# endernewton/tf-faster-rcnn

Hardware: NVIDIA H100
Metric: images/sec (higher is better)
Workload: dtype f16x3 (fp32-grade: fp16 hi/lo split of both operands, 3 wgmma f16 MMAs per product, fp32 accumulate)

## Files before the change

include/frcnn_b200.h:

```cpp
#ifndef FRCNN_B200_H_
#define FRCNN_B200_H_

#include <stddef.h>
#include <stdint.h>

#ifdef __cplusplus
extern "C" {
#endif

typedef enum {
  FRCNN_OK = 0,
  FRCNN_ERR_CUDA = -1,
  FRCNN_ERR_ARG = -2,
  FRCNN_ERR_NO_DEVICE = -3,
  FRCNN_ERR_DRIVER_ENTRY = -4,
  FRCNN_ERR_CAPACITY = -5
} frcnn_status;

#define FRCNN_NMS_PLUS_ONE 1u
#define FRCNN_NMS_INCLUSIVE 2u
#define FRCNN_NMS_SKIP_DEGENERATE 4u
#define FRCNN_NMS_MODE_CPU_NMS (FRCNN_NMS_PLUS_ONE | FRCNN_NMS_INCLUSIVE)
#define FRCNN_NMS_MODE_GPU_NMS (FRCNN_NMS_PLUS_ONE)
#define FRCNN_NMS_MODE_TF (FRCNN_NMS_SKIP_DEGENERATE)
// ... 16 lines not shown
int frcnn_nms_host(int* keep_out, int* num_out, const float* boxes_host, int boxes_num, int boxes_dim,
                   float nms_overlap_thresh, int device_id, unsigned flags);

int frcnn_nms_sorted_dev(const float* boxes_dev, int n, float thresh, unsigned flags, int max_out,
                         int* keep_dev, int* num_dev, void* stream);

typedef struct frcnn_conv_plan frcnn_conv_plan;
#define FRCNN_CONV_F16X3 0
#define FRCNN_CONV_TF32X3 1
#define FRCNN_CONV_F16X1 2

typedef struct {
  const float* in_dev;
  const void* w_hi_dev;
  const void* w_lo_dev;
  const float* scale_dev;
  const float* shift_dev;
  const float* residual_dev;
  float* out_dev;
  int n, h, w, cin;
  int cout, kh, kw, stride;
  int pad_t, pad_l;
  int ho, wo;
  int act;
  int block_n;
  int kb_per_chunk;
  int split_k;
  int impl;
  float out_mult;
  const float* in2_dev;
  int cin2;
  float* mean_dev;
  int mean_hw;
} frcnn_conv_desc;

int frcnn_conv_plan_create(frcnn_conv_plan** out, const frcnn_conv_desc* d);
int frcnn_conv_plan_run(const frcnn_conv_plan* p, void* stream);
int frcnn_conv_plan_geometry(const frcnn_conv_desc* d, int sm_count, int* out16);
int frcnn_conv_plan_info(const frcnn_conv_plan* p, int* block_n, int* tile_n, int* tile_h, int* tile_w,
                         int* grid_m, int* grid_n, int* splits, int* smem_bytes);
int frcnn_conv_plan_set_trace(frcnn_conv_plan* p, long long* trace_dev);
void frcnn_conv_plan_destroy(frcnn_conv_plan* p);
int frcnn_debug_watchdog(unsigned int* out16, int reset);

int frcnn_pack_conv_weights(const float* w_hwio_dev, void* w_hi_dev, void* w_lo_dev, int kh, int kw,
                            int cin, int cout, int wexp, void* stream);
int frcnn_pack_conv_weights_tf32(const float* w_hwio_dev, float* w_hi_dev, float* w_lo_dev, int kh, int kw,
                                 int cin, int cout, void* stream);

int frcnn_conv_first(const float* in_dev, const float* w_hwio_dev, const float* scale_dev,
                     const float* shift_dev, float* out_dev, int n, int h, int w, int cout, int k,
                     int stride, int pad_t, int pad_l, int ho, int wo, int act, void* stream);
int frcnn_depthwise3x3(const float* in_dev, const float* w_dev, const float* scale_dev,
                       const float* shift_dev, float* out_dev, int n, int h, int w, int c, int stride,
                       int pad_t, int pad_l, int ho, int wo, int act, void* stream);
int frcnn_max_pool(const float* in_dev, float* out_dev, int n, int h, int w, int c, int k, int stride,
                   int pad_t, int pad_l, int ho, int wo, int pad_is_neg_inf, void* stream);
int frcnn_spatial_mean(const float* in_dev, float* out_dev, int r, int hw, int c, void* stream);

int frcnn_preprocess(const unsigned char* img_dev, int h0, int w0, const double* means3, double fx, double fy,
                     float* blob_dev, int H, int W, void* stream);
int frcnn_preprocess_hflip(const unsigned char* img_dev, int h0, int w0, const double* means3, double fx, double fy,
                           float* blob_dev, int H, int W, void* stream);


int frcnn_rpn_decode(const float* rpn_out_dev, int ld, int delta_col, const float* base_anchors_dev, int num_anchors,
                     int batch, int fh, int fw, int feat_stride, float im_h, float im_w, float* scores_dev,
                     float* props_dev, void* stream);
size_t frcnn_sort_workspace_bytes(int n);
int frcnn_sort_desc(const float* keys_dev, int n, int batch, int* order_dev, float* sorted_keys_dev, void* workspace_dev,
                    size_t workspace_bytes, void* stream);
// ... 68 lines not shown
```

tf_faster_rcnn_b200/_native.py:

```python
import ctypes as C
import os

_HERE = os.path.dirname(os.path.abspath(__file__))
LIB_PATH = os.path.join(_HERE, "libfrcnn_b200_wd.so" if os.environ.get("FRCNN_LIB_VARIANT") == "wd" else "libfrcnn_b200.so")

NMS_PLUS_ONE, NMS_INCLUSIVE, NMS_SKIP_DEGENERATE = 1, 2, 4
NMS_MODE_CPU_NMS = NMS_PLUS_ONE | NMS_INCLUSIVE
NMS_MODE_GPU_NMS = NMS_PLUS_ONE
NMS_MODE_TF = NMS_SKIP_DEGENERATE
ACT_NONE, ACT_RELU, ACT_RELU6 = 0, 1, 2
CONV_F16X3, CONV_TF32X3, CONV_F16X1 = 0, 1, 2
SOFT_NMS_METHODS = {"linear": 0, "gaussian": 1, "hard": 2}
AUG_MAX_VIEWS = 16
BOX_VOTE_METHODS = {"ID": 0, "AVG": 1, "IOU_AVG": 2, "GENERALIZED_AVG": 3, "QUASI_SUM": 4, "TEMP_AVG": 5}
ROI_ALIGN_MAX_SAMPLING = 16
ROI_MAX_POOLED = 16

vp, ci, cf, cu, sz = C.c_void_p, C.c_int, C.c_float, C.c_uint, C.c_size_t
ip, fp = C.POINTER(C.c_int), C.POINTER(C.c_float)


class ConvDesc(C.Structure):
    _fields_ = [("in_dev", vp), ("w_hi_dev", vp), ("w_lo_dev", vp), ("scale_dev", vp), ("shift_dev", vp),
                ("residual_dev", vp), ("out_dev", vp),
                ("n", ci), ("h", ci), ("w", ci), ("cin", ci), ("cout", ci), ("kh", ci), ("kw", ci), ("stride", ci),
                ("pad_t", ci), ("pad_l", ci), ("ho", ci), ("wo", ci), ("act", ci), ("block_n", ci), ("kb_per_chunk", ci), ("split_k", ci),
                ("impl", ci), ("out_mult", cf), ("in2_dev", vp), ("cin2", ci), ("mean_dev", vp), ("mean_hw", ci)]


SIGNATURES = {
    "frcnn_version": (ci, []),
    "frcnn_last_error": (ci, [C.c_char_p, sz]),
    "frcnn_check_device": (ci, [ci]),
    "frcnn_zero_async": (ci, [vp, sz, vp]),
    "frcnn_graph_begin": (ci, [vp]),
    "frcnn_graph_end": (ci, [vp, C.POINTER(vp)]),
    "frcnn_graph_launch": (ci, [vp, vp]),
    "frcnn_graph_destroy": (None, [vp]),
    "frcnn_nms_host": (ci, [ip, ip, fp, ci, ci, cf, ci, cu]),
    "frcnn_nms_sorted_dev": (ci, [vp, ci, cf, cu, ci, vp, vp, vp]),
    "frcnn_conv_plan_create": (ci, [C.POINTER(vp), C.POINTER(ConvDesc)]),
    "frcnn_conv_plan_run": (ci, [vp, vp]),
    "frcnn_conv_plan_geometry": (ci, [C.POINTER(ConvDesc), ci, ip]),
    "frcnn_conv_plan_info": (ci, [vp, ip, ip, ip, ip, ip, ip, ip, ip]),
    "frcnn_conv_plan_set_trace": (ci, [vp, vp]),
    "frcnn_conv_plan_destroy": (None, [vp]),
    "frcnn_debug_watchdog": (ci, [C.POINTER(C.c_uint), ci]),
    "frcnn_pack_conv_weights": (ci, [vp, vp, vp, ci, ci, ci, ci, ci, vp]),
    "frcnn_pack_conv_weights_tf32": (ci, [vp, vp, vp, ci, ci, ci, ci, vp]),
    "frcnn_conv_first": (ci, [vp, vp, vp, vp, vp, ci, ci, ci, ci, ci, ci, ci, ci, ci, ci, ci, vp]),
    "frcnn_depthwise3x3": (ci, [vp, vp, vp, vp, vp, ci, ci, ci, ci, ci, ci, ci, ci, ci, ci, vp]),
    "frcnn_max_pool": (ci, [vp, vp, ci, ci, ci, ci, ci, ci, ci, ci, ci, ci, ci, vp]),
    "frcnn_spatial_mean": (ci, [vp, vp, ci, ci, ci, vp]),
    "frcnn_preprocess": (ci, [vp, ci, ci, C.POINTER(C.c_double), C.c_double, C.c_double, vp, ci, ci, vp]),
    "frcnn_rpn_decode": (ci, [vp, ci, ci, vp, ci, ci, ci, ci, ci, cf, cf, vp, vp, vp]),
    "frcnn_sort_workspace_bytes": (sz, [ci]),
    "frcnn_sort_desc": (ci, [vp, ci, ci, vp, vp, vp, sz, vp]),
    "frcnn_proposals": (ci, [vp, vp, vp, ci, ci, ci, ci, cf, cu, vp, vp, vp, vp, vp]),
    "frcnn_crop_pool": (ci, [vp, ci, ci, ci, ci, vp, ci, ci, ci, vp, vp]),
    "frcnn_roi_align": (ci, [vp, ci, ci, ci, ci, vp, ci, ci, cf, ci, ci, vp, vp]),
    "frcnn_roi_pool": (ci, [vp, ci, ci, ci, ci, vp, ci, ci, cf, vp, vp]),
    "frcnn_cls_finish": (ci, [vp, ci, ci, ci, fp, fp, vp, vp, vp, vp]),
    "frcnn_bbox_decode": (ci, [vp, vp, ci, ci, ci, vp, vp, vp]),
    "frcnn_detect_post_workspace_bytes": (sz, [ci, ci, ci]),
    "frcnn_detect_post": (ci, [vp, vp, vp, ci, ci, ci, cf, cf, cu, ci, ci, vp, vp, ci, vp, vp, vp, vp, sz, vp]),
    "frcnn_soft_nms_host": (ci, [fp, ip, ip, fp, ci, ci, ci, cf, cf, cf, ci]),
    "frcnn_detect_post_soft": (ci, [vp, vp, vp, ci, ci, ci, cf, ci, cf, cf, cf, ci, ci, vp, vp, ci, vp, vp, vp, vp, sz, vp]),
    "frcnn_detect_features": (ci, [vp, vp, vp, ci, ci, ci, ci, ci, vp, vp, vp]),
    "frcnn_detect_regions": (ci, [vp, vp, vp, vp, vp, ci, ci, ci, ci, cf, cu, cf, ci, ci, vp, vp, vp, vp, sz, vp, vp, vp, vp, vp, vp, vp,
                                  vp, vp]),
    "frcnn_boxes_to_rois": (ci, [vp, vp, vp, ci, ci, vp, vp, vp]),
    "frcnn_preprocess_hflip": (ci, [vp, ci, ci, C.POINTER(C.c_double), C.c_double, C.c_double, vp, ci, ci, vp]),
    "frcnn_aug_union": (ci, [C.POINTER(vp), C.POINTER(vp), C.POINTER(vp), ip, ip, ci, ci, ci, vp, vp, vp, vp, vp]),
    "frcnn_box_vote_host": (ci, [fp, fp, ci, ci, fp, ci, ci, cf, ci, cf, ci]),
    "frcnn_detect_post_vote": (ci, [vp, vp, vp, ci, ci, ci, cf, cf, cu, ci, ci, vp, vp, ci, vp, vp, vp, vp, sz, cf, ci, cf, vp, vp]),
    "frcnn_detect_post_soft_vote": (ci, [vp, vp, vp, ci, ci, ci, cf, ci, cf, cf, cf, ci, ci, vp, vp, ci, vp, vp, vp, vp, sz, cf, ci, cf, vp,
# ... 31 lines not shown
```

tf_faster_rcnn_b200/csrc/conv_gemm.cu:

```cuda
#include <cuda_fp16.h>
#include "common.cuh"
#include "../../include/frcnn_b200.h"
#include <stdlib.h>
#include <string.h>

namespace frcnn {

constexpr int BLOCK_M = 128;
constexpr int BLOCK_K = 32;
constexpr int A_TILE_BYTES = BLOCK_M * BLOCK_K * 4;
constexpr int NUM_CONSUMERS = 256;
constexpr int NUM_THREADS = NUM_CONSUMERS + 128;
constexpr int REGS_PRODUCER = 40, REGS_CONSUMER = 232;
constexpr int STAGES = 3;

struct ConvKernelParams {
  float* out;
  const float* residual;
  const float* scale;
  const float* shift;
  int cout, ho, wo, nimg;
  int tn, th, tw;
  int tiles_h, tiles_w;
  int kh, kw, cin, stride, pad_t, pad_l;
  int act;
  int a_box_bytes;
  int kb_per_split;
  int m_tiles, n_tiles, total_units, n_full, splits;
  int raster_n;
  float* ws;
  long long* trace;
  int num_kb_total;
  int cin2;
  float* mean_out;
  float* mean_ws;
  int mean_hw, mean_segs, mean_ld;
};

#ifdef FRCNN_WATCHDOG
#define FRCNN_TRACE(slot, kbv)                                                              \
  do {                                                                                      \
    if (p.trace && blockIdx.x == 0 && (kbv) < 64) p.trace[(kbv) * 8 + (slot)] = clock64(); \
  } while (0)
#else
#define FRCNN_TRACE(slot, kbv) do { } while (0)
#endif

template <int MODE> struct KTraits {
  static constexpr bool TF32 = MODE == FRCNN_CONV_TF32X3;
  static constexpr bool X1 = MODE == FRCNN_CONV_F16X1;
  static constexpr int BOXES = TF32 ? 1 : 2;
  static constexpr int A_BYTES = BOXES * A_TILE_BYTES;
  static constexpr float LO_SCALE = TF32 ? 1.f : 0.00048828125f;
};
template <int BN> constexpr int b_plane_bytes() { return BN * 128; }
template <int BN, int MODE> constexpr int stage_bytes() { return KTraits<MODE>::A_BYTES + 2 * b_plane_bytes<BN>(); }
template <int BN, int MODE> constexpr int smem_bytes() {
  return STAGES * stage_bytes<BN, MODE>() + 1024  + 64 ;
}
constexpr int MEAN_COLS = 64, MEAN_LD = MEAN_COLS + 2;
constexpr int MEAN_SMEM = BLOCK_M * MEAN_LD * 4;
static_assert(smem_bytes<128, FRCNN_CONV_F16X3>() + MEAN_SMEM <= 227 * 1024, "ring exceeds the sm_90 shared-memory limit per block");

struct Unit {
  int w0, h0, n0, nblk, z, kb0, num_kb, slot;
};
__device__ __forceinline__ Unit decode_unit(const ConvKernelParams& p, int u, int num_kb_total) {
  Unit t;
  int tile;
  if (u < p.n_full) { tile = u; t.z = 0; t.slot = -1; }
  else { const int v = u - p.n_full; t.slot = v / p.splits; t.z = v - t.slot * p.splits; tile = p.n_full + t.slot; }
  int mt;
  if (p.raster_n) { t.nblk = tile % p.n_tiles; mt = tile / p.n_tiles; }
  else { mt = tile % p.m_tiles; t.nblk = tile / p.m_tiles; }
  const int tile_w = mt % p.tiles_w;
  const int tile_h = (mt / p.tiles_w) % p.tiles_h;
  const int tile_n = mt / (p.tiles_w * p.tiles_h);
  t.w0 = tile_w * p.tw; t.h0 = tile_h * p.th; t.n0 = tile_n * p.tn;
  if (t.slot < 0) { t.kb0 = 0; t.num_kb = num_kb_total; }
  else { t.kb0 = t.z * p.kb_per_split; t.num_kb = min(p.kb_per_split, num_kb_total - t.kb0); }
  return t;
}

template <int ACT>
__device__ __forceinline__ float apply_act(float a) {
  if (ACT == FRCNN_ACT_RELU) return fmaxf(a, 0.f);
  if (ACT == FRCNN_ACT_RELU6) return fminf(fmaxf(a, 0.f), 6.f);
  return a;
}

template <bool RES, int ACT>
__device__ __forceinline__ float2 finish2(const float2 v, const float2 sc, const float2 sh, const float2 r) {
  float2 y;
  y.x = __fadd_rn(__fmul_rn(v.x, sc.x), sh.x); y.y = __fadd_rn(__fmul_rn(v.y, sc.y), sh.y);
  if (RES) { y.x = __fadd_rn(y.x, r.x); y.y = __fadd_rn(y.y, r.y); }
  y.x = apply_act<ACT>(y.x); y.y = apply_act<ACT>(y.y);
  return y;
}

constexpr int EPI_CHUNK = 8;
template <int BN, bool RES, int ACT>
__device__ __forceinline__ void epilogue_vec(const ConvKernelParams& p, const float (&acc)[BN / 2], const int cbase,
                                             const int pix0, const int pix1) {
  const int cout = p.cout;
  constexpr int NJ = BN / 8;
  constexpr int CH = NJ < EPI_CHUNK ? NJ : EPI_CHUNK;
  static_assert(NJ % CH == 0, "chunking");
  const float* const res0 = RES ? p.residual + (size_t)(pix0 >= 0 ? pix0 : 0) * cout : nullptr;
  const float* const res1 = RES ? p.residual + (size_t)(pix1 >= 0 ? pix1 : 0) * cout : nullptr;
#pragma unroll
  for (int j0 = 0; j0 < NJ; j0 += CH) {
    if (cbase + 8 * j0 >= cout) break;
    float2 sc[CH], sh[CH], r0[CH], r1[CH];
// ... 165 lines not shown
  uint8_t* smem = reinterpret_cast<uint8_t*>((reinterpret_cast<uintptr_t>(smem_raw) + 1023) & ~uintptr_t(1023));
  uint64_t* full = reinterpret_cast<uint64_t*>(smem + STAGES * kStage);
  uint64_t* empty = full + STAGES;

  const int warp = threadIdx.x >> 5;
  const int lane = threadIdx.x & 31;
  const int num_kb_total = p.num_kb_total;

  if (threadIdx.x == NUM_CONSUMERS) {
    tma_prefetch_desc(&tmA); tma_prefetch_desc(&tmBhi); tma_prefetch_desc(&tmBlo);
    if (p.cin2) tma_prefetch_desc(&tmA2);
    for (int s = 0; s < STAGES; ++s) { mbar_init(&full[s], 1); mbar_init(&empty[s], NUM_CONSUMERS); }
    mbar_fence_init();
  }
  __syncthreads();
  pdl_launch_dependents();
  pdl_wait();

  if (warp >= NUM_CONSUMERS / 32) {
    reg_dec<REGS_PRODUCER>();
    if (warp == NUM_CONSUMERS / 32 && lane == 0) {
      const int cchunks = p.cin / BLOCK_K;
      const int total1 = p.kh * p.kw * cchunks;
      const int cchunks2 = p.cin2 / BLOCK_K;
      const uint32_t tx = (uint32_t)(T::BOXES * p.a_box_bytes + (T::X1 ? 1 : 2) * kPlane);
      int s = 0; uint32_t ph = 0, kbt = 0;
      for (int u = blockIdx.x; u < p.total_units; u += gridDim.x) {
        const Unit t = decode_unit(p, u, num_kb_total);
#pragma unroll 1
        for (int kb = 0; kb < t.num_kb; ++kb, ++kbt) {
          MBAR_WAIT(&empty[s], ph ^ 1u, 4, kbt);
          uint8_t* st = smem + s * kStage;
          mbar_expect_tx(&full[s], tx);
#pragma unroll
          for (int i = 0; i < T::BOXES; ++i) {
            const int g32 = (t.kb0 + kb) * T::BOXES + i;
            int tap = g32 / cchunks, kc = g32 - tap * cchunks;
            const CUtensorMap* ma = &tmA;
            if (g32 >= total1) {
              tap = 0;
              if (cchunks2) { ma = &tmA2; kc = min(g32 - total1, cchunks2); }
              else kc = cchunks;
            }
            const int r = tap / p.kw, sx = tap - r * p.kw;
            tma_load_4d(st + i * A_TILE_BYTES, ma, &full[s], kc * BLOCK_K, t.w0 * p.stride + sx - p.pad_l,
                        t.h0 * p.stride + r - p.pad_t, t.n0);
          }
          const int kcoord = (t.kb0 + kb) * T::BOXES * BLOCK_K;
          tma_load_2d(st + T::A_BYTES, &tmBhi, &full[s], kcoord, t.nblk * BN);
          if (!T::X1) tma_load_2d(st + T::A_BYTES + kPlane, &tmBlo, &full[s], kcoord, t.nblk * BN);
          FRCNN_TRACE(0, kbt);
          if (++s == STAGES) { s = 0; ph ^= 1u; }
        }
      }
    }
    return;
  }

  reg_inc<REGS_CONSUMER>();
  const int wg = warp >> 2;
  const int q4 = lane & 3;
  const int r0 = wg * 64 + (warp & 3) * 16 + (lane >> 2);
  const uint32_t swz = (uint32_t)(lane >> 2);
  uint32_t aoff[4][2];
#pragma unroll
  for (int j = 0; j < 4; ++j)
#pragma unroll
    for (int h = 0; h < 2; ++h) {
      const int ch = T::TF32 ? j * 8 + h * 4 + q4 : (j & 1) * 16 + h * 8 + 2 * q4;
      const int box = T::TF32 ? 0 : j >> 1;
      aoff[j][h] = (uint32_t)(box * A_TILE_BYTES + r0 * 128) + ((((uint32_t)ch >> 2) ^ swz) << 4) + (((uint32_t)ch & 3u) << 2);
    }
  const uint32_t smem0 = smem_u32(smem);
  int s = 0; uint32_t ph = 0, kbt = 0;
  for (int u = blockIdx.x; u < p.total_units; u += gridDim.x) {
    const Unit t = decode_unit(p, u, num_kb_total);
    float acc[NACC], part[NACC];
#pragma unroll
    for (int i = 0; i < NACC; ++i) { acc[i] = 0.f; part[i] = 0.f; }
#pragma unroll 1
    for (int kb = 0; kb < t.num_kb; ++kb, ++kbt) {
// ... 227 lines not shown
  attr[0].val.programmaticStreamSerializationAllowed = 1;
  const bool pdl = pdl_enabled();
  cudaLaunchConfig_t cfg{};
  cfg.gridDim = p->grid; cfg.blockDim = dim3(NUM_THREADS); cfg.stream = st;
  cfg.dynamicSmemBytes = smem_bytes<BN, MODE>() + (p->kp.mean_out ? MEAN_SMEM : 0);
  cfg.attrs = attr; cfg.numAttrs = pdl ? 1 : 0;
  FRCNN_CUDA(cudaLaunchKernelEx(&cfg, conv_gemm_kernel<BN, MODE>, p->tmA, p->tmA2, p->tmBhi, p->tmBlo, p->kp));
  if (p->kp.mean_out) {
    cudaLaunchConfig_t mc{};
    const long n = (long)(p->kp.wo / p->kp.mean_hw) * p->kp.cout;
    mc.gridDim = dim3((unsigned)((n + 255) / 256)); mc.blockDim = dim3(256); mc.dynamicSmemBytes = 0; mc.stream = st;
    mc.attrs = attr; mc.numAttrs = pdl ? 1 : 0;
    FRCNN_CUDA(cudaLaunchKernelEx(&mc, mean_finish_kernel, p->kp));
  }
  if (p->n_tail > 0) {
    cudaLaunchConfig_t rc{};
    rc.gridDim = dim3((unsigned)(p->n_tail * (BLOCK_M / (256 / (BN / 4))))); rc.blockDim = dim3(256); rc.dynamicSmemBytes = 0; rc.stream = st;
    rc.attrs = attr; rc.numAttrs = pdl ? 1 : 0;
    FRCNN_CUDA(cudaLaunchKernelEx(&rc, tail_reduce_kernel<BN>, p->kp));
  }
  return OK;
}

struct Geometry {
  int n, h, w, ho, wo;
  int tn, th, tw, tiles_w, tiles_h, tiles_n;
  long m_tiles;
  int num_kb, bn, n_tiles, kpc;
  long tiles, n_tail;
  int splits, kbs;
  long total_units;
  int grid;
  int raster_n;
};

static int decide_geometry(const frcnn_conv_desc* d, int sms, Geometry* g) {
  FRCNN_REQUIRE(d->cin > 0 && d->cin % BLOCK_K == 0, "cin=%d must be a positive multiple of 32", d->cin);
  FRCNN_REQUIRE(d->kh >= 1 && d->kw >= 1 && d->stride >= 1 && d->stride <= 8, "bad filter geometry");
  FRCNN_REQUIRE(d->n > 0 && d->h > 0 && d->w > 0 && d->ho > 0 && d->wo > 0 && d->cout > 0, "bad shape");
  FRCNN_REQUIRE(sms > 0, "bad SM count");
  g->n = d->n; g->h = d->h; g->w = d->w; g->ho = d->ho; g->wo = d->wo;
  const bool pointwise = d->kh == 1 && d->kw == 1 && d->stride == 1 && d->pad_t == 0 && d->pad_l == 0 && g->ho == g->h && g->wo == g->w;
  const bool mean = d->mean_hw != 0;
  FRCNN_REQUIRE(d->cin2 >= 0 && d->cin2 % BLOCK_K == 0, "cin2=%d must be 0 or a positive multiple of 32", d->cin2);
  FRCNN_REQUIRE(d->cin2 == 0 || pointwise, "a second A source needs a pointwise layer (1x1, stride 1, no padding)");
  FRCNN_REQUIRE(!mean || pointwise, "the mean epilogue needs a pointwise layer (1x1, stride 1, no padding)");
  FRCNN_REQUIRE(!mean || d->cout % 4 == 0, "the mean epilogue needs cout %% 4 == 0 (cout=%d)", d->cout);
  FRCNN_REQUIRE(d->mean_hw >= 0 && (!mean || ((long)d->n * d->h * d->w) % d->mean_hw == 0),
                "mean_hw=%d must be positive and divide the pixel count", d->mean_hw);
  FRCNN_REQUIRE(!mean || d->split_k <= 1, "the mean epilogue is never split along K");
  if (pointwise) {
    g->w = g->wo = g->n * g->h * g->w; g->n = 1; g->h = g->ho = 1;
  }
  const int ktot = d->kh * d->kw * d->cin + d->cin2;
  choose_tile(g->n, g->ho, g->wo, d->stride, &g->tn, &g->th, &g->tw);
  g->tiles_w = cdiv(g->wo, g->tw); g->tiles_h = cdiv(g->ho, g->th); g->tiles_n = cdiv(g->n, g->tn);
  g->m_tiles = (long)g->tiles_w * g->tiles_h * g->tiles_n;
  const bool f16 = d->impl != FRCNN_CONV_TF32X3;
  const int ks = f16 ? 2 : 1;
  g->num_kb = cdiv(ktot / BLOCK_K, ks);
  g->kpc = d->kb_per_chunk > 0 ? d->kb_per_chunk : 8 / ks;
  int bn = d->block_n;
  if (bn == 0) {
    long best = -1;
    const int cands[2] = {128, 64};
    for (int i = 0; i < 2; ++i) {
      const int c = cands[i];
      if (c > 64 && c / 2 >= d->cout) continue;
      const long ctas = g->m_tiles * cdiv(d->cout, c);
      const long waves = (ctas + sms - 1) / sms;
      const long cost = f16 ? waves * (g->num_kb * 900L + 4000L) : waves * (g->num_kb * 1400L + 6000L);
      if (best < 0 || cost < best) { best = cost; bn = c; }
    }
  }
  FRCNN_REQUIRE(bn == 64 || bn == 128, "block_n must be 64 or 128");
  g->bn = bn;
  g->n_tiles = cdiv(d->cout, bn);
  g->tiles = g->m_tiles * g->n_tiles;
  FRCNN_REQUIRE(g->tiles <= 0x3fffffffL, "too many tiles");
  long n_tail = 0; int splits = 1;
  const int num_kb = g->num_kb;
  const int max_split = num_kb * ks / 8 < 8 ? num_kb * ks / 8 : 8;
  if (d->split_k > 1) {
    n_tail = g->tiles; splits = d->split_k;
  } else if (d->split_k == 0 && max_split >= 2) {
    const long rem = g->tiles % sms;
    if (g->tiles <= sms / 2) { if (num_kb * ks >= 16) { n_tail = g->tiles; splits = (int)(sms / g->tiles); } }
    else if (g->tiles > sms && rem > 0 && rem <= sms / 2 && num_kb * ks >= 48) { n_tail = rem; splits = (int)(sms / rem); }
    if (splits > max_split) splits = max_split;
    if (splits < 2) { n_tail = 0; splits = 1; }
  }
  int kbs = cdiv(num_kb, splits);
  splits = cdiv(num_kb, kbs);
  if (splits < 2 || (d->cout & 3) != 0 || mean) { n_tail = 0; splits = 1; kbs = num_kb; }
  FRCNN_REQUIRE(splits <= 64, "bad split_k");
  g->n_tail = n_tail; g->splits = splits; g->kbs = kbs;
  g->total_units = (g->tiles - n_tail) + n_tail * splits;
  FRCNN_REQUIRE(g->total_units <= 0x7fffffffL, "too many work units");
  g->grid = (int)(g->total_units < sms ? g->total_units : sms);
  {
    const char* e = getenv("FRCNN_CONV_RASTER");
    const double a_bytes = (double)d->n * d->h * d->w * (d->cin + d->cin2) * 4.0, b_bytes = (double)d->cout * ktot * 4.0;
    g->raster_n = (e && (e[0] == 'm' || e[0] == 'n')) ? (e[0] == 'n') : (a_bytes > b_bytes && g->n_tiles > 1);
  }
  return OK;
}

extern "C" int frcnn_conv_plan_geometry(const frcnn_conv_desc* d, int sm_count, int* out16) {
  FRCNN_REQUIRE(d && out16, "null argument");
  Geometry g;
  int rc = decide_geometry(d, sm_count, &g);
  if (rc) return rc;
  const int v[16] = {g.bn, g.tn, g.th, g.tw, (int)g.m_tiles, g.n_tiles, (int)g.tiles, (int)g.n_tail, g.splits, g.kbs,
                     (int)g.total_units, g.grid, g.num_kb, g.kpc, g.tiles_h, g.tiles_w};
  for (int i = 0; i < 16; ++i) out16[i] = v[i];
  return OK;
}

extern "C" int frcnn_conv_plan_create(frcnn_conv_plan** out, const frcnn_conv_desc* d) {
  FRCNN_REQUIRE(out && d, "null argument");
  FRCNN_REQUIRE(d->in_dev && d->w_hi_dev && d->w_lo_dev && (d->mean_hw ? d->mean_dev != nullptr : d->out_dev != nullptr),
                "null device pointer");
  FRCNN_REQUIRE(d->cin2 == 0 || d->in2_dev, "cin2=%d without in2_dev", d->cin2);
  int sms = 132;
  { int dev = 0; cudaDeviceProp pr; if (cudaGetDevice(&dev) == cudaSuccess && cudaGetDeviceProperties(&pr, dev) == cudaSuccess && pr.multiProcessorCount > 0) sms = pr.multiProcessorCount; }
  Geometry g;
  int grc = decide_geometry(d, sms, &g);
  if (grc) return grc;
  frcnn_conv_plan* p = (frcnn_conv_plan*)aligned_alloc(64, (sizeof(frcnn_conv_plan) + 63) / 64 * 64);
  if (!p) { set_error("out of host memory"); return ERR_ARG; }
  memset(p, 0, sizeof(*p));
  const int bn = g.bn;
  {
    uint64_t dims[4] = {(uint64_t)d->cin, (uint64_t)g.w, (uint64_t)g.h, (uint64_t)g.n};
    uint64_t strides[3] = {(uint64_t)d->cin * 4, (uint64_t)g.w * d->cin * 4, (uint64_t)g.h * g.w * d->cin * 4};
    uint32_t box[4] = {(uint32_t)BLOCK_K, (uint32_t)(g.tw * d->stride), (uint32_t)(g.th * d->stride), (uint32_t)g.tn};
    uint32_t es[4] = {1, (uint32_t)d->stride, (uint32_t)d->stride, 1};
    int rc = encode_map(&p->tmA, d->in_dev, 4, dims, strides, box, es);
    if (rc) { free(p); return rc; }
    p->tmA2 = p->tmA;
    if (d->cin2 > 0) {
      uint64_t dims2[4] = {(uint64_t)d->cin2, (uint64_t)g.w, (uint64_t)g.h, (uint64_t)g.n};
      uint64_t strides2[3] = {(uint64_t)d->cin2 * 4, (uint64_t)g.w * d->cin2 * 4, (uint64_t)g.h * g.w * d->cin2 * 4};
      rc = encode_map(&p->tmA2, d->in2_dev, 4, dims2, strides2, box, es);
      if (rc) { free(p); return rc; }
    }
  }
  const bool f16 = d->impl != FRCNN_CONV_TF32X3;
  {
    const uint64_t ktot = (uint64_t)d->kh * d->kw * d->cin + d->cin2;
    uint64_t dims[2] = {ktot, (uint64_t)d->cout};
    uint64_t strides[1] = {ktot * (f16 ? 2 : 4)};
    uint32_t box[2] = {(uint32_t)(f16 ? 2 * BLOCK_K : BLOCK_K), (uint32_t)bn};
    uint32_t es[2] = {1, 1};
    const CUtensorMapDataType dt = f16 ? CU_TENSOR_MAP_DATA_TYPE_FLOAT16 : CU_TENSOR_MAP_DATA_TYPE_FLOAT32;
    const CUtensorMapSwizzle sw = CU_TENSOR_MAP_SWIZZLE_128B;
    int rc = encode_map(&p->tmBhi, d->w_hi_dev, 2, dims, strides, box, es, dt, sw);
    if (!rc) rc = encode_map(&p->tmBlo, d->w_lo_dev, 2, dims, strides, box, es, dt, sw);
    if (rc) { free(p); return rc; }
  }
  ConvKernelParams& k = p->kp;
  k.out = d->out_dev; k.residual = d->residual_dev;
  k.cout = d->cout; k.ho = g.ho; k.wo = g.wo; k.nimg = g.n;
  k.tn = g.tn; k.th = g.th; k.tw = g.tw; k.tiles_h = g.tiles_h; k.tiles_w = g.tiles_w;
  k.kh = d->kh; k.kw = d->kw; k.cin = d->cin; k.stride = d->stride; k.pad_t = d->pad_t; k.pad_l = d->pad_l;
  k.act = d->act;
  k.a_box_bytes = g.tn * g.th * g.tw * BLOCK_K * 4;
  k.trace = nullptr;
  k.num_kb_total = g.num_kb;
  k.m_tiles = (int)g.m_tiles; k.n_tiles = g.n_tiles;
  k.kb_per_split = g.kbs; k.splits = g.splits; k.n_full = (int)(g.tiles - g.n_tail);
  k.total_units = (int)g.total_units;
  k.raster_n = g.raster_n;
  k.cin2 = d->cin2;
  k.mean_out = d->mean_hw ? d->mean_dev : nullptr; k.mean_ws = nullptr; k.mean_hw = d->mean_hw; k.mean_ld = g.n_tiles * bn;
  k.mean_segs = d->mean_hw ? (g.tw < cdiv(g.tw - 1, d->mean_hw) + 1 ? g.tw : cdiv(g.tw - 1, d->mean_hw) + 1) : 0;
  k.ws = nullptr; p->ws = nullptr; p->eff = nullptr; p->mean_ws = nullptr; p->n_tail = (int)g.n_tail;
  {
    const int padded = g.n_tiles * bn;
    const float om = f16 ? (d->out_mult != 0.f ? d->out_mult : 1.f) : 1.f;
    cudaError_t e = cudaMalloc(&p->eff, (size_t)2 * padded * sizeof(float));
    if (e != cudaSuccess) { free(p); return cuda_fail(e, "epilogue vectors", __FILE__, __LINE__); }
    prep_epilogue_vectors_kernel<<<cdiv(padded, 256), 256>>>(d->scale_dev, d->shift_dev, om, d->cout, padded, p->eff, p->eff + padded);
    e = cudaGetLastError();
    if (e == cudaSuccess) e = cudaDeviceSynchronize();
    if (e != cudaSuccess) { cudaFree(p->eff); free(p); return cuda_fail(e, "prep_epilogue_vectors", __FILE__, __LINE__); }
    k.scale = p->eff; k.shift = p->eff + padded;
  }
  if (g.n_tail > 0) {
    cudaError_t e = cudaMalloc(&p->ws, (size_t)g.n_tail * g.splits * BLOCK_M * bn * sizeof(float));
    if (e != cudaSuccess) { cudaFree(p->eff); free(p); return cuda_fail(e, "split-tile workspace", __FILE__, __LINE__); }
    k.ws = p->ws;
  }
  if (d->mean_hw) {
    cudaError_t e = cudaMalloc(&p->mean_ws, (size_t)g.m_tiles * k.mean_segs * k.mean_ld * sizeof(float));
    if (e != cudaSuccess) { cudaFree(p->eff); free(p); return cuda_fail(e, "mean workspace", __FILE__, __LINE__); }
    k.mean_ws = p->mean_ws;
  }
  p->grid = dim3((unsigned)g.grid, 1, 1);
  p->block_n = bn;
  p->impl = f16 ? (d->impl == FRCNN_CONV_F16X1 ? FRCNN_CONV_F16X1 : FRCNN_CONV_F16X3) : FRCNN_CONV_TF32X3;
  p->stages = STAGES;
  p->smem = f16 ? (bn == 128 ? smem_bytes<128, FRCNN_CONV_F16X3>() : smem_bytes<64, FRCNN_CONV_F16X3>())
              : (bn == 128 ? smem_bytes<128, FRCNN_CONV_TF32X3>() : smem_bytes<64, FRCNN_CONV_TF32X3>());
  if (d->mean_hw) p->smem += MEAN_SMEM;
  *out = p;
  return OK;
}

// ... 49 lines not shown
```

tf_faster_rcnn_b200/engine.py:

```python
import collections
import ctypes
import os

import numpy as np
import torch

from . import _native as N
from . import ops

F = np.float32
C_void = ctypes.c_void_p


def bn_fold(gamma, beta, mean, var, eps):
    inv = (gamma.astype(F) * (F(1.0) / np.sqrt(var.astype(F) + F(eps)))).astype(F)
    return inv, (beta.astype(F) - mean.astype(F) * inv).astype(F)


def concat_layers(weights, names, bn_eps):
    ss = [weights.scale_shift(nm, bn_eps) for nm in names]
    w = ops.concat_scaled_weights([weights[nm + "/weights"] for nm in names], [s for s, _ in ss])
    shift = ss[0][1]
    for _, sh in ss[1:]:
        shift = (shift + sh).astype(F)
# ... 73 lines not shown
        else:
            N.check(N.lib().frcnn_graph_launch(self._h, ops._stream()), "graph_launch")

    def __del__(self):
        try:
            if self._h:
                N.lib().frcnn_graph_destroy(self._h)
                self._h = ctypes.c_void_p()
        except Exception:
            pass


class Tape:
    def __init__(self, weights):
        self.w = weights
        self.steps = []
        self.flops = 0.0
        self.conv_flops = 0.0
        self.bufs = []
        self.conv_plans = []

    def new(self, *shape, dtype=torch.float32):
        t = torch.empty(shape, dtype=dtype, device="cuda")
        self.bufs.append(t)
        return t

    def add(self, label, fn):
        self.steps.append((label, fn))

    def run(self):
        for _, fn in self.steps:
            fn()

    def conv(self, x, name, stride=1, mode="SAME", act=N.ACT_RELU, bn_eps=None, residual=None, packed=None, x2=None, mean=False):
        pc = packed if packed is not None else self.w.packed_conv(name, bn_eps)
        n, h, w, _ = x.shape
        ho, wo, pt, pl = ops.conv_out_hw(h, w, pc.kh, stride, mode)
        out = self.new(n, pc.cout) if mean else self.new(n, ho, wo, pc.cout)
        plan = ops.ConvPlan(x, pc, out, stride, pt, pl, act, residual, x2=x2, mean=mean)
        self.conv_plans.append(plan)
        self.add("conv:" + name, plan.run)
        fl = 2.0 * n * ho * wo * pc.cout * pc.kh * pc.kw * pc.cin
        self.flops += fl
        self.conv_flops += fl
        return out

    def fc(self, x2d, name, act=N.ACT_NONE, packed=None):
        r, k = x2d.shape
        out = self.conv(x2d.view(1, 1, r, k), name, 1, "SAME", act, None, None, packed)
        return out.view(r, -1)

    def conv_first(self, x, name, k, stride, mode, act, bn_eps=None):
        sc, sh = self.w.scale_shift(name, bn_eps)
        wd = self.w.dev(name + "/weights", lambda: self.w[name + "/weights"])
        scd = None if sc is None else self.w.dev(name + "/scale", lambda: sc)
        shd = None if sh is None else self.w.dev(name + "/shift", lambda: sh)
        n, h, w, _ = x.shape
        ho, wo, pt, pl = ops.conv_out_hw(h, w, k, stride, mode)
        cout = int(self.w[name + "/weights"].shape[3])
        out = self.new(n, ho, wo, cout)
        self.add("conv_first:" + name, lambda: ops.conv_first(x, wd, scd, shd, out, k, stride, pt, pl, act))
        self.flops += 2.0 * n * ho * wo * cout * k * k * 3
        return out

    def depthwise(self, x, name, stride, act, bn_eps):
        sc, sh = self.w.scale_shift(name, bn_eps)
        c = x.shape[3]
        wd = self.w.dev(name + "/dw", lambda: self.w[name + "/depthwise_weights"].reshape(3, 3, c))
        scd = self.w.dev(name + "/scale", lambda: sc)
        shd = self.w.dev(name + "/shift", lambda: sh)
        n, h, w, _ = x.shape
        ho, wo, pt, pl = ops.conv_out_hw(h, w, 3, stride, "SAME" if stride == 1 else "EXPLICIT")
# ... 565 lines not shown
```

tf_faster_rcnn_b200/lib/nets/resnet_v1.py:

```python
from nets.network import Network
from tf_faster_rcnn_b200 import _native as N

_UNITS = {50: (3, 4, 6, 3), 101: (3, 4, 23, 3), 152: (3, 8, 36, 3)}
_EPS = 1e-5


class resnetv1(Network):
    def __init__(self, num_layers=50):
        Network.__init__(self)
        if num_layers not in _UNITS:
            raise NotImplementedError
        self._num_layers = num_layers
        self._scope = 'resnet_v1_%d' % num_layers
        n1, n2, n3, n4 = _UNITS[num_layers]
        self._blocks = [("block1", 64, [1] * (n1 - 1) + [2]), ("block2", 128, [1] * (n2 - 1) + [2]),
                        ("block3", 256, [1] * n3), ("block4", 512, [1] * n4)]

    def crop_pre_pool(self):
        return bool(self.options["resnet_max_pool"])

    def _bottleneck(self, t, x, prefix, base, stride, mean=False):
        depth = 4 * base
        r = t.conv(x, prefix + "/conv1", 1, "SAME", N.ACT_RELU, _EPS)
        r = t.conv(r, prefix + "/conv2", stride, "SAME" if stride == 1 else "EXPLICIT", N.ACT_RELU, _EPS)
        if x.shape[3] == depth:
            shortcut = x if stride == 1 else t.max_pool(x, 1, stride, "VALID")
            return t.conv(r, prefix + "/conv3", 1, "SAME", N.ACT_RELU, _EPS, residual=shortcut, mean=mean)
        assert stride == 1
        pc = t.w.packed_concat([prefix + "/conv3", prefix + "/shortcut"], _EPS)
        return t.conv(r, prefix + "/conv3", 1, "SAME", N.ACT_RELU, packed=pc, x2=x, mean=mean)

    def _run_blocks(self, t, x, blocks, mean_last=False):
        for bi, (bname, base, strides) in enumerate(blocks):
            for u, s in enumerate(strides, start=1):
                last = bi == len(blocks) - 1 and u == len(strides)
                x = self._bottleneck(t, x, "%s/%s/unit_%d/bottleneck_v1" % (self._scope, bname, u), base, s, mean_last and last)
        return x

    def _image_to_head(self, t, image):
        x = t.conv_first(image, self._scope + "/conv1", 7, 2, "EXPLICIT", N.ACT_RELU, _EPS)
        x = t.max_pool(x, 3, 2, "ZEROPAD1")
        x = self._run_blocks(t, x, self._blocks[:3])
        self._layers['head'] = x
        return x

    def _head_to_tail(self, t, pool5):
        return self._run_blocks(t, pool5, self._blocks[3:], mean_last=True)
```

tf_faster_rcnn_b200/ops.py:

```python
import ctypes as C
import os

import numpy as np
import torch

from . import _native as N


def _stream():
    return C.c_void_p(torch.cuda.current_stream().cuda_stream)


def _p(t):
    return C.c_void_p(t.data_ptr()) if t is not None else C.c_void_p(0)


def _f32(t):
    assert t.dtype == torch.float32 and t.is_cuda and t.is_contiguous(), "expected contiguous cuda fp32"
    return t


def zeros(shape, dtype=torch.float32):
    t = torch.empty(shape, dtype=dtype, device="cuda")
    N.check(N.lib().frcnn_zero_async(_p(t), t.numel() * t.element_size(), _stream()), "zero_async")
# ... 24 lines not shown
        w = torch.from_numpy(wnp).cuda()
        if w.dim() == 2:
            w = w.view(1, 1, w.shape[0], w.shape[1])
        self.kh, self.kw, self.cin, self.cout = (int(v) for v in w.shape)
        ktot = self.kh * self.kw * self.cin
        self.impl = conv_impl() if impl is None else impl
        if self.impl in (N.CONV_F16X3, N.CONV_F16X1):
            self.wexp = weight_exponent(wnp)
            self.out_mult = float(np.ldexp(1.0, -self.wexp))
            self.w_hi = torch.empty((self.cout, ktot), dtype=torch.float16, device="cuda")
            self.w_lo = torch.empty_like(self.w_hi)
            N.check(N.lib().frcnn_pack_conv_weights(_p(w), _p(self.w_hi), _p(self.w_lo), self.kh, self.kw, self.cin,
                                                    self.cout, self.wexp, _stream()), "pack_conv_weights")
        else:
            self.wexp, self.out_mult = 0, 1.0
            self.w_hi = torch.empty((self.cout, ktot), dtype=torch.float32, device="cuda")
            self.w_lo = torch.empty_like(self.w_hi)
            N.check(N.lib().frcnn_pack_conv_weights_tf32(_p(w), _p(self.w_hi), _p(self.w_lo), self.kh, self.kw, self.cin,
                                                         self.cout, _stream()), "pack_conv_weights_tf32")
        torch.cuda.current_stream().synchronize()
        self.scale = None if scale is None else torch.as_tensor(np.ascontiguousarray(scale), dtype=torch.float32).cuda()
        self.shift = None if shift is None else torch.as_tensor(np.ascontiguousarray(shift), dtype=torch.float32).cuda()


def concat_scaled_weights(ws, scales):
    parts = []
    for w, s in zip(ws, scales):
        w = np.asarray(w, dtype=np.float32)
        assert w.ndim == 4 and w.shape[:2] == (1, 1), w.shape
        parts.append(w if s is None else (w * np.asarray(s, dtype=np.float32)).astype(np.float32))
    return np.ascontiguousarray(np.concatenate(parts, axis=2))


class ConvPlan:

    def __init__(self, x, pc, out, stride=1, pad_t=0, pad_l=0, act=N.ACT_NONE, residual=None, block_n=0, kb_per_chunk=0, split_k=0,
                 x2=None, mean=False):
        _f32(x); _f32(out)
        n, h, w, cin = x.shape
        cin2 = 0
        if x2 is not None:
            _f32(x2)
            assert x2.shape[:3] == x.shape[:3], (x2.shape, x.shape)
            cin2 = int(x2.shape[3])
        assert cin + cin2 == pc.cin, (cin, cin2, pc.cin)
        if mean:
            ho, wo = h, w
            assert tuple(out.shape) == (n, pc.cout), (out.shape, n, pc.cout)
        else:
            no, ho, wo, co = out.shape
            assert no == n and co == pc.cout
        d = N.ConvDesc(_p(x), _p(pc.w_hi), _p(pc.w_lo), _p(pc.scale), _p(pc.shift), _p(residual), _p(None if mean else out),
                       n, h, w, cin, pc.cout, pc.kh, pc.kw, stride, pad_t, pad_l, ho, wo, act, block_n, kb_per_chunk, split_k,
                       pc.impl, pc.out_mult, _p(x2), cin2, _p(out if mean else None), h * w if mean else 0)
        self._h = C.c_void_p()
        N.check(N.lib().frcnn_conv_plan_create(C.byref(self._h), C.byref(d)), "conv_plan_create")
        self._keep = (x, pc, out, residual, x2)
        self.flops = 2.0 * n * ho * wo * pc.cout * pc.kh * pc.kw * pc.cin

    def run(self):
        N.check(N.lib().frcnn_conv_plan_run(self._h, _stream()), "conv_plan_run")

    def info(self):
        v = [C.c_int() for _ in range(8)]
        N.check(N.lib().frcnn_conv_plan_info(self._h, *[C.byref(a) for a in v]), "conv_plan_info")
        return dict(zip(["block_n", "tile_n", "tile_h", "tile_w", "grid_m", "grid_n", "splits", "smem"], [a.value for a in v]))

    def __del__(self):
        try:
            if self._h:
                N.lib().frcnn_conv_plan_destroy(self._h)
                self._h = C.c_void_p()
        except Exception:
            pass


def conv_out_hw(h, w, k, stride, mode):
    if mode == "SAME":
        pt, _ = same_pads(h, k, stride)
        pl, _ = same_pads(w, k, stride)
        return -(-h // stride), -(-w // stride), pt, pl
    pb = (k - 1) // 2
    return (h + k - 1 - k) // stride + 1, (w + k - 1 - k) // stride + 1, pb, pb


def conv_first(x, w_hwio_dev, scale, shift, out, k, stride, pad_t, pad_l, act):
    n, h, w, _ = x.shape
# ... 206 lines not shown
```

Baseline: 262.7.

## Skip padding-only conv taps per output position in per-ROI tail convs

Adds a roi_taps mode to the implicit-GEMM conv: each M tile covers one spatial position across many ROIs (tn=BLOCK_M, th=tw=1). For that position it loads only the kernel taps that land inside the image, and skips k-blocks that would read only zero padding. It is enabled automatically for the stride-1 3x3 conv2 layers in the ResNet head-to-tail blocks when the counted live k-blocks are fewer than in the full plan. The cost is a different tiling (one pixel per tile, no split-K, raster_n forced), which may lower reuse of the A tile and change load balance.

```diff
diff --git a/include/frcnn_b200.h b/include/frcnn_b200.h
--- a/include/frcnn_b200.h
+++ b/include/frcnn_b200.h
@@ -72,11 +72,13 @@
   int cin2;
   float* mean_dev;
   int mean_hw;
+  int roi_taps;
 } frcnn_conv_desc;
 
 int frcnn_conv_plan_create(frcnn_conv_plan** out, const frcnn_conv_desc* d);
 int frcnn_conv_plan_run(const frcnn_conv_plan* p, void* stream);
 int frcnn_conv_plan_geometry(const frcnn_conv_desc* d, int sm_count, int* out16);
+int frcnn_conv_plan_live_k_blocks(const frcnn_conv_desc* d, int sm_count, long long* k_blocks);
 int frcnn_conv_plan_info(const frcnn_conv_plan* p, int* block_n, int* tile_n, int* tile_h, int* tile_w,
                          int* grid_m, int* grid_n, int* splits, int* smem_bytes);
 int frcnn_conv_plan_set_trace(frcnn_conv_plan* p, long long* trace_dev);
diff --git a/tf_faster_rcnn_b200/_native.py b/tf_faster_rcnn_b200/_native.py
--- a/tf_faster_rcnn_b200/_native.py
+++ b/tf_faster_rcnn_b200/_native.py
@@ -25,7 +25,8 @@
                 ("residual_dev", vp), ("out_dev", vp),
                 ("n", ci), ("h", ci), ("w", ci), ("cin", ci), ("cout", ci), ("kh", ci), ("kw", ci), ("stride", ci),
                 ("pad_t", ci), ("pad_l", ci), ("ho", ci), ("wo", ci), ("act", ci), ("block_n", ci), ("kb_per_chunk", ci), ("split_k", ci),
-                ("impl", ci), ("out_mult", cf), ("in2_dev", vp), ("cin2", ci), ("mean_dev", vp), ("mean_hw", ci)]
+                ("impl", ci), ("out_mult", cf), ("in2_dev", vp), ("cin2", ci), ("mean_dev", vp), ("mean_hw", ci),
+                ("roi_taps", ci)]
 
 
 SIGNATURES = {
@@ -42,6 +43,7 @@
     "frcnn_conv_plan_create": (ci, [C.POINTER(vp), C.POINTER(ConvDesc)]),
     "frcnn_conv_plan_run": (ci, [vp, vp]),
     "frcnn_conv_plan_geometry": (ci, [C.POINTER(ConvDesc), ci, ip]),
+    "frcnn_conv_plan_live_k_blocks": (ci, [C.POINTER(ConvDesc), ci, C.POINTER(C.c_longlong)]),
     "frcnn_conv_plan_info": (ci, [vp, ip, ip, ip, ip, ip, ip, ip, ip]),
     "frcnn_conv_plan_set_trace": (ci, [vp, vp]),
     "frcnn_conv_plan_destroy": (None, [vp]),
diff --git a/tf_faster_rcnn_b200/csrc/conv_gemm.cu b/tf_faster_rcnn_b200/csrc/conv_gemm.cu
--- a/tf_faster_rcnn_b200/csrc/conv_gemm.cu
+++ b/tf_faster_rcnn_b200/csrc/conv_gemm.cu
@@ -3,6 +3,7 @@
 #include "../../include/frcnn_b200.h"
 #include <stdlib.h>
 #include <string.h>
+#include <algorithm>
 
 namespace frcnn {
 
@@ -35,6 +36,7 @@
   float* mean_out;
   float* mean_ws;
   int mean_hw, mean_segs, mean_ld;
+  int roi_taps, kb_per_tap;
 };
 
 #ifdef FRCNN_WATCHDOG
@@ -64,6 +66,7 @@
 
 struct Unit {
   int w0, h0, n0, nblk, z, kb0, num_kb, slot;
+  int tap_r, tap_s, taps_w;
 };
 __device__ __forceinline__ Unit decode_unit(const ConvKernelParams& p, int u, int num_kb_total) {
   Unit t;
@@ -79,6 +82,13 @@
   t.w0 = tile_w * p.tw; t.h0 = tile_h * p.th; t.n0 = tile_n * p.tn;
   if (t.slot < 0) { t.kb0 = 0; t.num_kb = num_kb_total; }
   else { t.kb0 = t.z * p.kb_per_split; t.num_kb = min(p.kb_per_split, num_kb_total - t.kb0); }
+  if (p.roi_taps) {
+    t.tap_r = max(p.pad_t - t.h0, 0);
+    t.tap_s = max(p.pad_l - t.w0, 0);
+    const int taps_h = max(min(p.kh, p.ho + p.pad_t - t.h0) - t.tap_r, 0);
+    t.taps_w = max(min(p.kw, p.wo + p.pad_l - t.w0) - t.tap_s, 0);
+    t.num_kb = taps_h * t.taps_w * p.kb_per_tap;
+  }
   return t;
 }
 
@@ -310,9 +320,14 @@
           MBAR_WAIT(&empty[s], ph ^ 1u, 4, kbt);
           uint8_t* st = smem + s * kStage;
           mbar_expect_tx(&full[s], tx);
+          int gkb = t.kb0 + kb;
+          if (p.roi_taps) {
+            const int lt = kb / p.kb_per_tap, rr = lt / t.taps_w;
+            gkb = ((t.tap_r + rr) * p.kw + t.tap_s + (lt - rr * t.taps_w)) * p.kb_per_tap + (kb - lt * p.kb_per_tap);
+          }
 #pragma unroll
           for (int i = 0; i < T::BOXES; ++i) {
-            const int g32 = (t.kb0 + kb) * T::BOXES + i;
+            const int g32 = gkb * T::BOXES + i;
             int tap = g32 / cchunks, kc = g32 - tap * cchunks;
             const CUtensorMap* ma = &tmA;
             if (g32 >= total1) {
@@ -324,7 +339,7 @@
             tma_load_4d(st + i * A_TILE_BYTES, ma, &full[s], kc * BLOCK_K, t.w0 * p.stride + sx - p.pad_l,
                         t.h0 * p.stride + r - p.pad_t, t.n0);
           }
-          const int kcoord = (t.kb0 + kb) * T::BOXES * BLOCK_K;
+          const int kcoord = gkb * T::BOXES * BLOCK_K;
           tma_load_2d(st + T::A_BYTES, &tmBhi, &full[s], kcoord, t.nblk * BN);
           if (!T::X1) tma_load_2d(st + T::A_BYTES + kPlane, &tmBlo, &full[s], kcoord, t.nblk * BN);
           FRCNN_TRACE(0, kbt);
@@ -618,6 +633,8 @@
   long total_units;
   int grid;
   int raster_n;
+  int kb_per_tap;
+  long live_kb;
 };
 
 static int decide_geometry(const frcnn_conv_desc* d, int sms, Geometry* g) {
@@ -635,16 +652,26 @@
   FRCNN_REQUIRE(d->mean_hw >= 0 && (!mean || ((long)d->n * d->h * d->w) % d->mean_hw == 0),
                 "mean_hw=%d must be positive and divide the pixel count", d->mean_hw);
   FRCNN_REQUIRE(!mean || d->split_k <= 1, "the mean epilogue is never split along K");
-  if (pointwise) {
+  const bool f16 = d->impl != FRCNN_CONV_TF32X3;
+  const int ks = f16 ? 2 : 1;
+  const bool roi = d->roi_taps != 0;
+  if (roi) {
+    FRCNN_REQUIRE(d->stride == 1 && d->ho == d->h && d->wo == d->w, "roi_taps needs stride 1 and an output the size of the input");
+    FRCNN_REQUIRE(!d->residual_dev && d->cin2 == 0 && !mean, "roi_taps takes no residual, second source or mean epilogue");
+    FRCNN_REQUIRE(d->split_k <= 1, "roi_taps is never split along K (split_k=%d)", d->split_k);
+    FRCNN_REQUIRE(d->cin % (BLOCK_K * ks) == 0, "roi_taps needs whole k-blocks per tap: cin=%d must be a multiple of %d", d->cin,
+                  BLOCK_K * ks);
+  }
+  if (pointwise && !roi) {
     g->w = g->wo = g->n * g->h * g->w; g->n = 1; g->h = g->ho = 1;
   }
   const int ktot = d->kh * d->kw * d->cin + d->cin2;
-  choose_tile(g->n, g->ho, g->wo, d->stride, &g->tn, &g->th, &g->tw);
+  if (roi) { g->tn = BLOCK_M; g->th = g->tw = 1; }
+  else choose_tile(g->n, g->ho, g->wo, d->stride, &g->tn, &g->th, &g->tw);
   g->tiles_w = cdiv(g->wo, g->tw); g->tiles_h = cdiv(g->ho, g->th); g->tiles_n = cdiv(g->n, g->tn);
   g->m_tiles = (long)g->tiles_w * g->tiles_h * g->tiles_n;
-  const bool f16 = d->impl != FRCNN_CONV_TF32X3;
-  const int ks = f16 ? 2 : 1;
   g->num_kb = cdiv(ktot / BLOCK_K, ks);
+  g->kb_per_tap = roi ? d->cin / (BLOCK_K * ks) : 0;
   g->kpc = d->kb_per_chunk > 0 ? d->kb_per_chunk : 8 / ks;
   int bn = d->block_n;
   if (bn == 0) {
@@ -667,7 +694,8 @@
   long n_tail = 0; int splits = 1;
   const int num_kb = g->num_kb;
   const int max_split = num_kb * ks / 8 < 8 ? num_kb * ks / 8 : 8;
-  if (d->split_k > 1) {
+  if (roi) {
+  } else if (d->split_k > 1) {
     n_tail = g->tiles; splits = d->split_k;
   } else if (d->split_k == 0 && max_split >= 2) {
     const long rem = g->tiles % sms;
@@ -689,6 +717,18 @@
     const double a_bytes = (double)d->n * d->h * d->w * (d->cin + d->cin2) * 4.0, b_bytes = (double)d->cout * ktot * 4.0;
     g->raster_n = (e && (e[0] == 'm' || e[0] == 'n')) ? (e[0] == 'n') : (a_bytes > b_bytes && g->n_tiles > 1);
   }
+  g->live_kb = g->tiles * (long)num_kb;
+  if (roi) {
+    g->raster_n = 1;
+    long taps = 0;
+    for (int y = 0; y < g->ho; ++y)
+      for (int x = 0; x < g->wo; ++x) {
+        const int th = std::min(d->kh, g->ho + d->pad_t - y) - std::max(d->pad_t - y, 0);
+        const int tw = std::min(d->kw, g->wo + d->pad_l - x) - std::max(d->pad_l - x, 0);
+        taps += (long)std::max(th, 0) * std::max(tw, 0);
+      }
+    g->live_kb = taps * g->kb_per_tap * g->tiles_n * g->n_tiles;
+  }
   return OK;
 }
 
@@ -700,6 +740,15 @@
   const int v[16] = {g.bn, g.tn, g.th, g.tw, (int)g.m_tiles, g.n_tiles, (int)g.tiles, (int)g.n_tail, g.splits, g.kbs,
                      (int)g.total_units, g.grid, g.num_kb, g.kpc, g.tiles_h, g.tiles_w};
   for (int i = 0; i < 16; ++i) out16[i] = v[i];
+  return OK;
+}
+
+extern "C" int frcnn_conv_plan_live_k_blocks(const frcnn_conv_desc* d, int sm_count, long long* k_blocks) {
+  FRCNN_REQUIRE(d && k_blocks, "null argument");
+  Geometry g;
+  int rc = decide_geometry(d, sm_count, &g);
+  if (rc) return rc;
+  *k_blocks = g.live_kb;
   return OK;
 }
 
@@ -761,6 +810,7 @@
   k.cin2 = d->cin2;
   k.mean_out = d->mean_hw ? d->mean_dev : nullptr; k.mean_ws = nullptr; k.mean_hw = d->mean_hw; k.mean_ld = g.n_tiles * bn;
   k.mean_segs = d->mean_hw ? (g.tw < cdiv(g.tw - 1, d->mean_hw) + 1 ? g.tw : cdiv(g.tw - 1, d->mean_hw) + 1) : 0;
+  k.roi_taps = d->roi_taps != 0; k.kb_per_tap = g.kb_per_tap;
   k.ws = nullptr; p->ws = nullptr; p->eff = nullptr; p->mean_ws = nullptr; p->n_tail = (int)g.n_tail;
   {
     const int padded = g.n_tiles * bn;
diff --git a/tf_faster_rcnn_b200/engine.py b/tf_faster_rcnn_b200/engine.py
--- a/tf_faster_rcnn_b200/engine.py
+++ b/tf_faster_rcnn_b200/engine.py
@@ -129,12 +129,14 @@
         for _, fn in self.steps:
             fn()
 
-    def conv(self, x, name, stride=1, mode="SAME", act=N.ACT_RELU, bn_eps=None, residual=None, packed=None, x2=None, mean=False):
+    def conv(self, x, name, stride=1, mode="SAME", act=N.ACT_RELU, bn_eps=None, residual=None, packed=None, x2=None, mean=False,
+             per_roi=False):
         pc = packed if packed is not None else self.w.packed_conv(name, bn_eps)
         n, h, w, _ = x.shape
         ho, wo, pt, pl = ops.conv_out_hw(h, w, pc.kh, stride, mode)
         out = self.new(n, pc.cout) if mean else self.new(n, ho, wo, pc.cout)
-        plan = ops.ConvPlan(x, pc, out, stride, pt, pl, act, residual, x2=x2, mean=mean)
+        plan = ops.ConvPlan(x, pc, out, stride, pt, pl, act, residual, x2=x2, mean=mean,
+                            roi_taps="auto" if per_roi else False)
         self.conv_plans.append(plan)
         self.add("conv:" + name, plan.run)
         fl = 2.0 * n * ho * wo * pc.cout * pc.kh * pc.kw * pc.cin
diff --git a/tf_faster_rcnn_b200/lib/nets/resnet_v1.py b/tf_faster_rcnn_b200/lib/nets/resnet_v1.py
--- a/tf_faster_rcnn_b200/lib/nets/resnet_v1.py
+++ b/tf_faster_rcnn_b200/lib/nets/resnet_v1.py
@@ -19,10 +19,10 @@
     def crop_pre_pool(self):
         return bool(self.options["resnet_max_pool"])
 
-    def _bottleneck(self, t, x, prefix, base, stride, mean=False):
+    def _bottleneck(self, t, x, prefix, base, stride, mean=False, per_roi=False):
         depth = 4 * base
         r = t.conv(x, prefix + "/conv1", 1, "SAME", N.ACT_RELU, _EPS)
-        r = t.conv(r, prefix + "/conv2", stride, "SAME" if stride == 1 else "EXPLICIT", N.ACT_RELU, _EPS)
+        r = t.conv(r, prefix + "/conv2", stride, "SAME" if stride == 1 else "EXPLICIT", N.ACT_RELU, _EPS, per_roi=per_roi)
         if x.shape[3] == depth:
             shortcut = x if stride == 1 else t.max_pool(x, 1, stride, "VALID")
             return t.conv(r, prefix + "/conv3", 1, "SAME", N.ACT_RELU, _EPS, residual=shortcut, mean=mean)
@@ -30,11 +30,12 @@
         pc = t.w.packed_concat([prefix + "/conv3", prefix + "/shortcut"], _EPS)
         return t.conv(r, prefix + "/conv3", 1, "SAME", N.ACT_RELU, packed=pc, x2=x, mean=mean)
 
-    def _run_blocks(self, t, x, blocks, mean_last=False):
+    def _run_blocks(self, t, x, blocks, mean_last=False, per_roi=False):
         for bi, (bname, base, strides) in enumerate(blocks):
             for u, s in enumerate(strides, start=1):
                 last = bi == len(blocks) - 1 and u == len(strides)
-                x = self._bottleneck(t, x, "%s/%s/unit_%d/bottleneck_v1" % (self._scope, bname, u), base, s, mean_last and last)
+                x = self._bottleneck(t, x, "%s/%s/unit_%d/bottleneck_v1" % (self._scope, bname, u), base, s, mean_last and last,
+                                     per_roi)
         return x
 
     def _image_to_head(self, t, image):
@@ -45,4 +46,4 @@
         return x
 
     def _head_to_tail(self, t, pool5):
-        return self._run_blocks(t, pool5, self._blocks[3:], mean_last=True)
+        return self._run_blocks(t, pool5, self._blocks[3:], mean_last=True, per_roi=True)
diff --git a/tf_faster_rcnn_b200/ops.py b/tf_faster_rcnn_b200/ops.py
--- a/tf_faster_rcnn_b200/ops.py
+++ b/tf_faster_rcnn_b200/ops.py
@@ -80,10 +80,17 @@
     return np.ascontiguousarray(np.concatenate(parts, axis=2))
 
 
+def live_k_blocks(d):
+    kb = C.c_longlong()
+    N.check(N.lib().frcnn_conv_plan_live_k_blocks(C.byref(d), torch.cuda.get_device_properties(torch.cuda.current_device())
+                                                  .multi_processor_count, C.byref(kb)), "conv_plan_live_k_blocks")
+    return kb.value
+
+
 class ConvPlan:
 
     def __init__(self, x, pc, out, stride=1, pad_t=0, pad_l=0, act=N.ACT_NONE, residual=None, block_n=0, kb_per_chunk=0, split_k=0,
-                 x2=None, mean=False):
+                 x2=None, mean=False, roi_taps=False):
         _f32(x); _f32(out)
         n, h, w, cin = x.shape
         cin2 = 0
@@ -101,6 +108,14 @@
         d = N.ConvDesc(_p(x), _p(pc.w_hi), _p(pc.w_lo), _p(pc.scale), _p(pc.shift), _p(residual), _p(None if mean else out),
                        n, h, w, cin, pc.cout, pc.kh, pc.kw, stride, pad_t, pad_l, ho, wo, act, block_n, kb_per_chunk, split_k,
                        pc.impl, pc.out_mult, _p(x2), cin2, _p(out if mean else None), h * w if mean else 0)
+        if roi_taps == "auto":
+            if os.environ.get("FRCNN_CONV_ROI_TAPS", "1") != "0":
+                full = live_k_blocks(d)
+                d.roi_taps = 1
+                d.roi_taps = int(live_k_blocks(d) < full)
+        else:
+            d.roi_taps = int(bool(roi_taps))
+        self.roi_taps = bool(d.roi_taps)
         self._h = C.c_void_p()
         N.check(N.lib().frcnn_conv_plan_create(C.byref(self._h), C.byref(d)), "conv_plan_create")
         self._keep = (x, pc, out, residual, x2)
```

After: 265.3 (median of 6 runs). About the same (+1.0%).
